# Enigmatisms/NeRF

Measured on AMD Instinct MI355X. Metric: rays/s (64+128 samples), 800x800, higher is better.
Workload: dtype bf16

## Files before the change

### nerf_amd/csrc/host_common.h

```cpp
#pragma once
#include <hip/hip_runtime.h>
#include <mutex>
#include <vector>

namespace nerf_host {

inline std::mutex& table_mutex() { static std::mutex m; return m; }

inline int current_device() {
    int dev = 0;
    if (hipGetDevice(&dev) != hipSuccess) dev = 0;
    return dev;
}

inline int allow_dynamic_lds(const void* fn, size_t lds) {
    struct Entry { int dev; const void* fn; size_t lds; };
    static std::vector<Entry> done;
    const int dev = current_device();
    std::lock_guard<std::mutex> lock(table_mutex());
    for (auto& e : done)
        if (e.dev == dev && e.fn == fn) {
            if (e.lds >= lds) return 0;
            hipError_t err = hipFuncSetAttribute(fn, hipFuncAttributeMaxDynamicSharedMemorySize, (int)lds);
            if (err != hipSuccess) return (int)err;
            e.lds = lds;
            return 0;
        }
    hipError_t err = hipFuncSetAttribute(fn, hipFuncAttributeMaxDynamicSharedMemorySize, (int)lds);
    if (err != hipSuccess) return (int)err;
    done.push_back({dev, fn, lds});
    return 0;
}

inline int cu_count() {
    static int n_cu[64] = {0};
    const int dev = current_device();
    std::lock_guard<std::mutex> lock(table_mutex());
    int& slot = n_cu[dev & 63];
    if (!slot) {
        hipDeviceProp_t p;
        slot = (hipGetDeviceProperties(&p, dev) == hipSuccess && p.multiProcessorCount > 0) ? p.multiProcessorCount : 256;
    }
    return slot;
}

}
```

### nerf_amd/csrc/mlp_kernels.hip

```cpp
#include "mlp_core.h"
#include "launchers.h"

namespace {

template <class P, int L, int NKG>
DEVINL void encode(float x, float y, float z, int h, typename P::BReg (&B)[NKG]) {
    if constexpr (P::FAST_PE) {
        float sv[3], cv[3];
        sincos_quadrant(x, sv[0], cv[0]); sincos_quadrant(y, sv[1], cv[1]); sincos_quadrant(z, sv[2], cv[2]);
#pragma unroll
        for (int f = 0; f < L; ++f) {
#pragma unroll
            for (int c = 0; c < 3; ++c) {
                const int q = 3 * f + c;
                P::set(B[q >> 3], q & 7, h ? cv[c] : sv[c]);
                if (f + 1 < L) {
                    const float s2 = 2.0f * sv[c];
                    const float ns = s2 * cv[c];
                    const float nc = __builtin_fmaf(-s2, sv[c], 1.0f);
                    sv[c] = ns; cv[c] = nc;
                }
            }
        }
#pragma unroll
// ... 233 lines not shown
    split_sample_index(s, m0, q, r);
    n = wave_uniform(q); si0 = __builtin_amdgcn_readfirstlane(r);
}
template <bool EXPLICIT_Z>
DEVINL Sample fetch_ray_sample(const nerf_amd_samples& s, int64_t n, int si) {
    Sample r;
    const float* ry = s.rays + n * 6;
    const float ox = ry[0], oy = ry[1], oz = ry[2];
    r.dx = ry[3]; r.dy = ry[4]; r.dz = ry[5];
    float zv;
    if (EXPLICIT_Z || s.z) zv = s.z[n * s.z_stride + si];
    else {
        const float uu = s.u ? s.u[n * s.S + si] : philox_u_strat(s.rng_seed, n + s.rng_ray_offset, si);
        zv = s.z_base[si] + uu * s.z_jitter;
    }
    r.x = ox + zv * r.dx; r.y = oy + zv * r.dy; r.z = oz + zv * r.dz;
    return r;
}

struct PropResident {
    using R = ResidentSet<PropLayout::N_FRAGS, 32, 0, 168, MLP_RES_PROP_HOLE>;
    static constexpr int NSLOT = MLP_RES_PROP_NSLOT;
    static constexpr uint32_t RING = NSLOT * MLP_CHUNK_BYTES, BIAS = RING, RES = RING + 9216, TOTAL = RES + R::N * 1024;
    static_assert(TOTAL <= 160 * 1024, "LDS");
};
struct MipResident {
    using R = ResidentSet<MipLayout::N_FRAGS, 32, MLP_RES_MIP_TAIL>;
    static constexpr int NSLOT = MLP_RES_MIP_NSLOT;
    static constexpr uint32_t RING = NSLOT * MLP_CHUNK_BYTES, BIAS = RING, STASH = BIAS + MipLayout::N_BIAS * 4, DIR = STASH + 4 * 2 * 4 * 1024,
                              RES = DIR + 4 * 2 * 1024, TOTAL = RES + R::N * 1024;
    static_assert(TOTAL <= 160 * 1024, "LDS");
};

DEVINL void load_biases(const void* packed, size_t stream_bytes, int n_bias, uint32_t lds_off = MLP_RING_BYTES) {
    const float* b = reinterpret_cast<const float*>(reinterpret_cast<const char*>(packed) + stream_bytes);
    float* dst = reinterpret_cast<float*>(smem + lds_off);
    for (int i = threadIdx.x; i < n_bias; i += blockDim.x) dst[i] = b[i];
    __syncthreads();
}

struct ActDump {
    char* base;
    unsigned long long layer_stride;
    char* mask_base;
    unsigned long long mask_layer_stride;
};
template <class P>
DEVINL void dump_breg(const ActDump& d, int layer, int64_t subtile, int kg, int lane, const typename P::BReg& r) {
#ifndef ABL_NODUMPST
    P::store_global(d.base + (size_t)layer * d.layer_stride + ((size_t)subtile * 16 + kg) * (size_t)P::BREG_LDS, lane, r);
#endif
}

template <class P> constexpr uint32_t lds_maskacc() { return lds_total<P>(); }
template <class P> constexpr uint32_t lds_total_train() { return lds_total<P>() + P::NW * 2 * P::NT * 1024; }
template <class P> constexpr uint32_t lds_scaleacc() { return lds_total_train<P>(); }
template <class P> constexpr uint32_t lds_total_train_f8() { return lds_total_train<P>() + P::NW * 2 * P::NT * 1024; }
template <class P, bool F8>
DEVINL void dump_hidden(const ActDump& d, uint32_t sacc_wave, int layer, int64_t subtile, int t, int kg, int lane, const typename P::BReg& r) {
    if constexpr (F8) {
        const uint32_t E = f8_group_exponent<false>(r);
        f8_store_group(d.base + (size_t)layer * d.layer_stride + (size_t)subtile * F8_SUB_BYTES, kg, lane, f8_encode_group(r, E), E,
                       sacc_wave + ((layer & 1) * P::NT + t) * 1024);
    } else {
        dump_breg<P>(d, layer, subtile, kg, lane, r);
    }
// ... 14 lines not shown
DEVINL uint32_t breg_bits(const f32x8& v) {
    uint32_t m = 0;
#pragma unroll
    for (int e = 0; e < 8; ++e) m |= (v[e] > 0.0f ? 1u : 0u) << ((e >> 1) + 16 * (e & 1));
    return m;
}
template <class P>
DEVINL void mask_or(uint32_t acc_wave, int layer, int t, int kg, int lane, const typename P::BReg& v) {
    unsigned* w = reinterpret_cast<unsigned*>(smem + acc_wave + ((layer & 1) * P::NT + t) * 1024 + lane * 16 + (kg >> 2) * 4);
    __hip_atomic_fetch_or(w, breg_bits(v) << (4 * (kg & 3)), __ATOMIC_RELAXED, __HIP_MEMORY_SCOPE_WORKGROUP);
}
template <class P, bool F8 = false>
DEVINL void mask_flush(const ActDump& d, uint32_t acc_wave, int layer, int64_t sub0, int lane, uint32_t sacc_wave = 0) {
    asm volatile("" ::: "memory");
#pragma unroll
    for (int t = 0; t < P::NT; ++t) {
        f32x4* rec = reinterpret_cast<f32x4*>(smem + acc_wave + ((layer & 1) * P::NT + t) * 1024 + lane * 16);
        const f32x4 v = *rec;
        *reinterpret_cast<f32x4*>(d.mask_base + (size_t)layer * d.mask_layer_stride + (size_t)(sub0 + t) * 1024 + lane * 16) = v;
        *rec = f32x4{0.0f, 0.0f, 0.0f, 0.0f};
        if constexpr (F8)
            f8_flush_scales(d.base + (size_t)layer * d.layer_stride + (size_t)(sub0 + t) * F8_SUB_BYTES, lane, sacc_wave + ((layer & 1) * P::NT + t) * 1024);
    }
    asm volatile("" ::: "memory");
}
template <class P>
DEVINL void mask_acc_init(uint32_t acc_wave, int lane) {
#pragma unroll
    for (int i = 0; i < 2 * P::NT; ++i) *reinterpret_cast<f32x4*>(smem + acc_wave + i * 1024 + lane * 16) = f32x4{0.0f, 0.0f, 0.0f, 0.0f};
}

template <class P, bool TRAIN, bool F8 = false>
__global__ __launch_bounds__(P::NW * 64) void proposal_kernel(const void* __restrict__ packed, nerf_amd_samples s,
                                                              float* __restrict__ density, ActDump dump) {
    using L = PropLayout;
    using BReg = typename P::BReg;
    constexpr int FPC = P::FPC;
    constexpr bool RES = MLP_RESIDENT_PROP && wide_bf16<P>() && !TRAIN;
    using R = typename conditional_type<RES, PropResident::R, NoResident>::type;
    using WS = typename conditional_type<RES, WeightStream<P, PropResident::NSLOT, R, PropResident::RES>, WeightStream<P, MLP_NSLOT>>::type;
    constexpr uint32_t bias0 = RES ? PropResident::BIAS : MLP_RING_BYTES;
    load_biases(packed, L::stream_bytes(P::PREC), L::N_BIAS, bias0);
    WS ws;
    ws.init(packed, (L::N_FRAGS - R::N) / FPC);
    const int lane = lane_id(), h = lane >> 5, j = lane & 31;
    const int wave = __builtin_amdgcn_readfirstlane((int)(threadIdx.x >> 6));
    constexpr int NT = P::NT;
    constexpr int TS = P::NW * NT * 32;
    const int64_t n_tiles = (s.M + TS - 1) / TS;
    const uint32_t macc = lds_maskacc<P>() + wave * 2 * NT * 1024;
    const uint32_t sacc = lds_scaleacc<P>() + wave * 2 * NT * 1024;
    if constexpr (TRAIN) mask_acc_init<P>(macc, lane);

    for (int64_t tile = blockIdx.x; tile < n_tiles; tile += gridDim.x) {
        int64_t m[NT];
        BReg enc[NT][4];
        if constexpr (ray_tile<P>::value) {
            static_assert(NT == 2 && P::FAST_PE && !TRAIN, "the ray tile is an inference form of the wide bf16 tile");
            const int64_t m0 = tile * TS + wave * 64;
            int64_t n; int si0;
            split_wave_index(s, m0 < s.M ? m0 : s.M - 64, n, si0);
            const Sample sm = fetch_ray_sample<false>(s, n, si0 + lane);
            encode_pair<P, 10, 4>(sm.x, sm.y, sm.z, enc[0], enc[1]);
            half_swap_groups<4>(enc[0], enc[1]);
        } else if constexpr (NT == 2 && P::FAST_PE) {
            m[0] = tile * TS + (wave * NT) * 32 + j;
            m[1] = m[0] + 32;
            const int64_t mo = h ? m[1] : m[0];
            const Sample sm = fetch_sample(s, mo < s.M ? mo : s.M - 1, false);
            encode_pair<P, 10, 4>(sm.x, sm.y, sm.z, enc[0], enc[1]);
            half_swap_groups<4>(enc[0], enc[1]);
            if constexpr (TRAIN) {
#pragma unroll
                for (int t = 0; t < NT; ++t)
#pragma unroll
                    for (int k = 0; k < 4; ++k) dump_breg<P>(dump, 4, tile * (TS / 32) + wave * NT + t, k, lane, enc[t][k]);
            }
        } else {
#pragma unroll
        for (int t = 0; t < NT; ++t) {
            m[t] = tile * TS + (wave * NT + t) * 32 + j;
            const Sample sm = fetch_sample(s, m[t] < s.M ? m[t] : s.M - 1, false);
            encode<P, 10, 4>(sm.x, sm.y, sm.z, h, enc[t]);
            if constexpr (TRAIN) {
#pragma unroll
                for (int k = 0; k < 4; ++k) dump_breg<P>(dump, 4, tile * (TS / 32) + wave * NT + t, k, lane, enc[t][k]);
            }
        }
        }
        BReg a[NT][16], b[NT][16];
        int lay = 0, lay_pend = 0;
        const int64_t sub0 = tile * (TS / 32) + wave * NT;
        auto put = [&](BReg (&buf)[NT][16], int layer, int fb, int t, const f32x16& acc, int half) {
            buf[t][2 * fb + half] = to_breg_half<P, true>(acc, half);
            if constexpr (TRAIN) {
                dump_hidden<P, F8>(dump, sacc, layer, sub0 + t, t, 2 * fb + half, lane, buf[t][2 * fb + half]);
                mask_or<P>(macc, layer, t, 2 * fb + half, lane, buf[t][2 * fb + half]);
            }
        };
        auto OA = [&](int fb, int t, const f32x16& acc, int half) { put(a, lay, fb, t, acc, half); };
        auto OB = [&](int fb, int t, const f32x16& acc, int half) { put(b, lay, fb, t, acc, half); };
        auto OA_pend = [&](int fb, int t, const f32x16& acc, int half) { put(a, lay_pend, fb, t, acc, half); };
        auto OB_pend = [&](int fb, int t, const f32x16& acc, int half) { put(b, lay_pend, fb, t, acc, half); };
        auto IN_A = [&](int kg, int t) -> BReg { return a[t][kg]; };
        Deferred<P, 6, 2> d = dense<P, 4, 8, L::START[0]>(ws, bias0 + L::BIAS_OFF[0] * 4,
            [&](int kg, int t) -> BReg { return enc[t][kg]; }, OA, NoPrev{});
        static_assert(same_stream_shape<R, FPC>(L::START[1], L::START[3], 128 + P::DEPTH), "chunk parity (in stream space) of the shared a -> b instance");
        auto IN_B = [&](int kg, int t) -> BReg { return b[t][kg]; };
#pragma unroll 1
        for (int r = 0; r < 2; ++r) {
            lay_pend = lay; lay = 1 + 2 * r;
            d = dense<P, 16, 8, L::START[1]>(ws, bias0 + (L::BIAS_OFF[1] + r * 512) * 4, IN_A, OB, prev_of(d, OA_pend));
            if constexpr (TRAIN) mask_flush<P, F8>(dump, macc, lay_pend, sub0, lane, sacc);
            if (r == 0) {
                lay_pend = lay; lay = 2;
                d = dense<P, 16, 8, L::START[2]>(ws, bias0 + L::BIAS_OFF[2] * 4, IN_B, OA, prev_of(d, OB_pend));
                if constexpr (TRAIN) mask_flush<P, F8>(dump, macc, lay_pend, sub0, lane, sacc);
            }
        }
        lay_pend = lay;
        float dens[NT];
        auto OH = [&](int, int t, const f32x16& acc, int half) { if (half == 0) dens[t] = acc[0]; };
        dense<P, 16, 1, L::START[4]>(ws, bias0 + L::BIAS_OFF[4] * 4, IN_B, OH, prev_of(d, OB_pend)).flush(OH);
        if constexpr (TRAIN) mask_flush<P, F8>(dump, macc, lay_pend, sub0, lane, sacc);
#pragma unroll
        for (int t = 0; t < NT; ++t) {
            if constexpr (ray_tile<P>::value) {
                const int64_t m0 = tile * TS + wave * 64;
                if (h == 0 && m0 < s.M) density[m0 + t * 32 + j] = dens[t];
            } else {
                if (h == 0 && m[t] < s.M) density[m[t]] = dens[t];
            }
        }
    }
    ws.drain();
}

constexpr uint32_t lds_total_narrow() { return MLP_RING_BYTES + 9216; }
template <class P>
__global__ __launch_bounds__(P::NW * 64) void proposal128_kernel(const void* __restrict__ packed, nerf_amd_samples s, float* __restrict__ density) {
    using L = PropLayout128;
    using BReg = typename P::BReg;
    constexpr int HK = L::HK, HFB = L::HFB;
    load_biases(packed, L::stream_bytes(P::PREC), L::N_BIAS);
    WeightStream<P, MLP_NSLOT> ws;
    ws.init(packed, L::N_FRAGS / P::FPC);
    const int lane = lane_id(), h = lane >> 5, j = lane & 31;
    const int wave = __builtin_amdgcn_readfirstlane((int)(threadIdx.x >> 6));
    constexpr int NT = P::NT;
    constexpr int TS = P::NW * NT * 32;
    const int64_t n_tiles = (s.M + TS - 1) / TS;
    const uint32_t bias0 = MLP_RING_BYTES;
    for (int64_t tile = blockIdx.x; tile < n_tiles; tile += gridDim.x) {
        int64_t m[NT];
        BReg a[NT][HK], b[NT][HK];
        auto OA = [&](int fb, int t, const f32x16& acc, int half) { a[t][2 * fb + half] = to_breg_half<P, true>(acc, half); };
        auto OB = [&](int fb, int t, const f32x16& acc, int half) { b[t][2 * fb + half] = to_breg_half<P, true>(acc, half); };
        auto IN_A = [&](int kg, int t) -> BReg { return a[t][kg]; };
        auto IN_B = [&](int kg, int t) -> BReg { return b[t][kg]; };
        Deferred<P, HFB - 2, 2> d;
        {
            BReg enc[NT][4];
            constexpr int PAIRED = (NT >= 2 && P::FAST_PE) ? 2 : 0;
#pragma unroll
            for (int t = 0; t < NT; ++t) m[t] = tile * TS + (wave * NT + t) * 32 + j;
            if constexpr (PAIRED) {
                const int64_t mo = h ? m[1] : m[0];
                const Sample sm = fetch_sample(s, mo < s.M ? mo : s.M - 1, false);
// ... 1 lines not shown
                half_swap_groups<4>(enc[0], enc[1]);
            }
#pragma unroll
            for (int t = PAIRED; t < NT; ++t) {
                const Sample sm = fetch_sample(s, m[t] < s.M ? m[t] : s.M - 1, false);
                encode<P, 10, 4>(sm.x, sm.y, sm.z, h, enc[t]);
            }
            d = dense<P, 4, HFB, L::START[0]>(ws, bias0 + L::BIAS_OFF[0] * 4, [&](int kg, int t) -> BReg { return enc[t][kg]; }, OA, NoPrev{});
        }
        d = dense<P, HK, HFB, L::START[1]>(ws, bias0 + L::BIAS_OFF[1] * 4, IN_A, OB, prev_of(d, OA));
        d = dense<P, HK, HFB, L::START[2]>(ws, bias0 + L::BIAS_OFF[2] * 4, IN_B, OA, prev_of(d, OB));
        d = dense<P, HK, HFB, L::START[3]>(ws, bias0 + L::BIAS_OFF[3] * 4, IN_A, OB, prev_of(d, OA));
        float dens[NT];
        auto OH = [&](int, int t, const f32x16& acc, int half) { if (half == 0) dens[t] = acc[0]; };
        dense<P, HK, 1, L::START[4]>(ws, bias0 + L::BIAS_OFF[4] * 4, IN_B, OH, prev_of(d, OB)).flush(OH);
        skip_frags<P, L::USED_FRAGS, L::N_FRAGS - L::USED_FRAGS>(ws);
#pragma unroll
        for (int t = 0; t < NT; ++t)
            if (h == 0 && m[t] < s.M) density[m[t]] = dens[t];
    }
    ws.drain();
}

struct FusedComposite {
    float* rgb;
    float* depth;
    float* weights;
    int white_bkg;
    float near, far;
};

template <class P, bool TRAIN, bool IPE = false, bool F8 = false, bool FUSED = false>
__global__ __launch_bounds__(P::NW * 64) void mip_kernel(const void* __restrict__ packed, nerf_amd_samples s,
                                                         float* __restrict__ rgbo, FusedComposite fc, ActDump dump) {
    using L = MipLayout;
    using BReg = typename P::BReg;
    constexpr int FPC = P::FPC;
#ifdef MLP_CLOCKPROBE
    const uint64_t probe_c0 = __builtin_readcyclecounter(), probe_r0 = __builtin_amdgcn_s_memrealtime();
#endif
    if constexpr (FUSED) { if (threadIdx.x < 16) reinterpret_cast<unsigned*>(smem + lds_tile<P>() + P::NW * P::NT * 32 * 32 + P::NW * P::NT * 8)[threadIdx.x] = 0u; }
    constexpr bool RES = MLP_RESIDENT_MIP && wide_bf16<P>() && !TRAIN && !IPE && !F8 && !FUSED;
    using R = typename conditional_type<RES, MipResident::R, NoResident>::type;
    using WS = typename conditional_type<RES, WeightStream<P, MipResident::NSLOT, R, MipResident::RES>, WeightStream<P, MLP_NSLOT>>::type;
    constexpr uint32_t bias0 = RES ? MipResident::BIAS : LDS_BIAS;
    constexpr uint32_t stash_lds = RES ? MipResident::STASH : LDS_STASH, dirs_lds = RES ? MipResident::DIR : lds_dir<P>();
    load_biases(packed, L::stream_bytes(P::PREC), L::N_BIAS, bias0);
    WS ws;
    ws.init(packed, (L::N_FRAGS - R::N) / FPC);
    const int lane = lane_id(), h = lane >> 5, j = lane & 31;
    const int wave = __builtin_amdgcn_readfirstlane((int)(threadIdx.x >> 6));
    constexpr int NT = P::NT;
    constexpr int TS = P::NW * NT * 32;
    const int64_t n_tiles = (s.M + TS - 1) / TS;
    const uint32_t macc = lds_maskacc<P>() + wave * 2 * NT * 1024;
    const uint32_t sacc = lds_scaleacc<P>() + wave * 2 * NT * 1024;
    if constexpr (TRAIN) mask_acc_init<P>(macc, lane);
    const uint32_t enc_lds0 = stash_lds + wave * NT * 4 * P::BREG_LDS + lane * 16;
    const uint32_t dir_lds0 = dirs_lds + wave * NT * 1024 + lane * 16;
    auto enc_lds = [&](int t) -> uint32_t { return enc_lds0 + t * 4 * P::BREG_LDS; };
    auto dir_lds = [&](int t) -> uint32_t { return dir_lds0 + t * 1024; };

    for (int64_t tile = blockIdx.x; tile < n_tiles; tile += gridDim.x) {
        int64_t m[NT];
        BReg a[NT][16], b[NT][16];
        int lay = 0, lay_pend = 0;
        const int64_t sub0 = tile * (TS / 32) + wave * NT;
        auto put = [&](BReg (&buf)[NT][16], int layer, int fb, int t, const f32x16& acc, int half) {
            buf[t][2 * fb + half] = to_breg_half<P, true>(acc, half);
            if constexpr (TRAIN) {
                dump_hidden<P, F8>(dump, sacc, layer, sub0 + t, t, 2 * fb + half, lane, buf[t][2 * fb + half]);
                mask_or<P>(macc, layer, t, 2 * fb + half, lane, buf[t][2 * fb + half]);
            }
        };
        auto OA = [&](int fb, int t, const f32x16& acc, int half) { put(a, lay, fb, t, acc, half); };
        auto OB = [&](int fb, int t, const f32x16& acc, int half) { put(b, lay, fb, t, acc, half); };
        auto OA_pend = [&](int fb, int t, const f32x16& acc, int half) { put(a, lay_pend, fb, t, acc, half); };
        auto OB_pend = [&](int fb, int t, const f32x16& acc, int half) { put(b, lay_pend, fb, t, acc, half); };
        auto IN_A = [&](int kg, int t) -> BReg { return a[t][kg]; };
        Deferred<P, 6, 2> d;
        {
            BReg enc[NT][4];
            if constexpr (ray_tile<P>::value) {
                static_assert(NT == 2 && P::FAST_PE && !TRAIN && !IPE && !F8 && !FUSED, "the ray tile is an inference form of the wide bf16 tile");
                const int64_t m0 = tile * TS + wave * 64;
                int64_t n; int si0;
                const int64_t m0c = m0 < s.M ? m0 : s.M - 64;
                split_wave_index(s, m0c, n, si0);
                const BReg* row = reinterpret_cast<const BReg*>(reinterpret_cast<const char*>(rgbo + m0c * 4) + h * (DIR_TABLE_ROW / 2));
                const BReg row0 = row[0], row1 = row[1];
                const Sample sm = fetch_ray_sample<true>(s, n, si0 + lane);
                P::stash(dir_lds(0), row0);
                P::stash(dir_lds(1), row1);
                encode_pair<P, 10, 4>(sm.x, sm.y, sm.z, enc[0], enc[1]);
                half_swap_groups<4>(enc[0], enc[1]);
#pragma unroll
                for (int t = 0; t < NT; ++t) {
#pragma unroll
                    for (int k = 0; k < 4; ++k) P::stash(enc_lds(t) + k * P::BREG_LDS, enc[t][k]);
                }
            } else if constexpr (NT == 2 && P::FAST_PE && !IPE && !FUSED) {
                m[0] = tile * TS + (wave * NT) * 32 + j;
                m[1] = m[0] + 32;
                const int64_t mo = h ? m[1] : m[0];
                const Sample sm = fetch_sample(s, mo < s.M ? mo : s.M - 1, true);
                encode_pair<P, 10, 4>(sm.x, sm.y, sm.z, enc[0], enc[1]);
                half_swap_groups<4>(enc[0], enc[1]);
                uint32_t d0[3] = {__builtin_bit_cast(uint32_t, sm.dx), __builtin_bit_cast(uint32_t, sm.dy), __builtin_bit_cast(uint32_t, sm.dz)};
                uint32_t d1[3] = {d0[0], d0[1], d0[2]};
#pragma unroll
                for (int c = 0; c < 3; ++c) half_swap(d0[c], d1[c]);
#pragma unroll
                for (int t = 0; t < NT; ++t) {
#pragma unroll
                    for (int k = 0; k < 4; ++k) P::stash(enc_lds(t) + k * P::BREG_LDS, enc[t][k]);
                    if constexpr (TRAIN) {
#pragma unroll
                        for (int k = 0; k < 4; ++k) dump_breg<P>(dump, 8, sub0 + t, k, lane, enc[t][k]);
                    }
                    const uint32_t* dd = t ? d1 : d0;
                    const f32x4 dv = {__builtin_bit_cast(float, dd[0]), __builtin_bit_cast(float, dd[1]), __builtin_bit_cast(float, dd[2]), 0.0f};
                    *reinterpret_cast<f32x4*>(smem + dir_lds(t)) = dv;
                }
            } else {
#pragma unroll
            for (int t = 0; t < NT; ++t) {
                m[t] = tile * TS + (wave * NT + t) * 32 + j;
                Sample sm;
                if constexpr (IPE) {
                    const IpeSample is = fetch_sample_ipe(s, m[t] < s.M ? m[t] : s.M - 1);
                    encode_ipe<P, 10, 4>(is.mu, is.var, h, enc[t]);
                    sm.dx = is.dx; sm.dy = is.dy; sm.dz = is.dz;
                } else {
                    sm = fetch_sample(s, m[t] < s.M ? m[t] : s.M - 1, true);
                    encode<P, 10, 4>(sm.x, sm.y, sm.z, h, enc[t]);
                }
#pragma unroll
                for (int k = 0; k < 4; ++k) P::stash(enc_lds(t) + k * P::BREG_LDS, enc[t][k]);
                if constexpr (TRAIN) {
#pragma unroll
                    for (int k = 0; k < 4; ++k) dump_breg<P>(dump, 8, sub0 + t, k, lane, enc[t][k]);
                }
                f32x4 dv = {sm.dx, sm.dy, sm.dz, 0.0f};
                if constexpr (FUSED) {
                    const int64_t mm_ = m[t] < s.M ? m[t] : s.M - 1;
                    const int64_t n_ = mm_ / s.S;
                    const int si_ = (int)(mm_ - n_ * s.S);
                    const float nrm_ = norm3(sm.dx, sm.dy, sm.dz);
                    const float* zz_ = s.z + n_ * s.z_stride;
                    const float zn0 = zz_[si_] * nrm_;
                    const float dl = (si_ + 1 < s.S) ? (zz_[si_ + 1] * nrm_ - zn0) : 1e10f;
                    dv[3] = h ? dl : zn0;
                }
                *reinterpret_cast<f32x4*>(smem + dir_lds(t)) = dv;
            }
            }
            d = dense<P, 4, 8, L::START[0]>(ws, bias0 + L::BIAS_OFF[0] * 4,
                [&](int kg, int t) -> BReg { return enc[t][kg]; }, OA, NoPrev{});
        }
        static_assert(same_stream_shape<R, FPC>(L::START[1], L::START[3], 128 + P::DEPTH) && same_stream_shape<R, FPC>(L::START[1], L::START[5], 128 + P::DEPTH) &&
                      same_stream_shape<R, FPC>(L::START[2], L::START[6], 128 + P::DEPTH) && L::BIAS_OFF[6] == 6 * 256, "uniform layer loop (chunk parity in stream space)");
        auto IN_B = [&](int kg, int t) -> BReg { return b[t][kg]; };
#pragma unroll 1
        for (int r = 0; r < 3; ++r) {
            lay_pend = lay; lay = 1 + 2 * r;
            d = dense<P, 16, 8, L::START[1]>(ws, bias0 + (1 + 2 * r) * 256 * 4, IN_A, OB, prev_of(d, OA_pend));
            if constexpr (TRAIN) mask_flush<P, F8>(dump, macc, lay_pend, sub0, lane, sacc);
            lay_pend = lay; lay = 2 + 2 * r;
            if (r == 1) {
                d = dense<P, 20, 8, L::START[4]>(ws, bias0 + L::BIAS_OFF[4] * 4,
                    [&](int kg, int t) -> BReg { if (kg < 4) return P::unstash(enc_lds(t) + kg * P::BREG_LDS); return b[t][kg >= 4 ? kg - 4 : 0]; },
                    OA, prev_of(d, OB_pend));
            } else {
                d = dense<P, 16, 8, L::START[2]>(ws, bias0 + (2 + 2 * r) * 256 * 4, IN_B, OA, prev_of(d, OB_pend));
            }
            if constexpr (TRAIN) mask_flush<P, F8>(dump, macc, lay_pend, sub0, lane, sacc);
        }
        lay_pend = lay;
        float sigma[NT];
        auto OSIG = [&](int, int t, const f32x16& acc, int half) { if (half == 0) sigma[t] = acc[0]; };
        const auto dsig = dense<P, 16, 1, L::START[7]>(ws, bias0 + L::BIAS_OFF[7] * 4, IN_A, OSIG, prev_of(d, OA_pend));
        if constexpr (TRAIN) mask_flush<P, F8>(dump, macc, 6, sub0, lane, sacc);
        BReg denc[NT][2];
        if constexpr (ray_tile<P>::value) {
        } else {
#pragma unroll
        for (int t = 0; t < NT; ++t) {
            const f32x4 dv = *reinterpret_cast<const f32x4*>(smem + dir_lds(t));
            const float nrm = norm3(dv[0], dv[1], dv[2]);
// ... 94 lines not shown
                    const int q = base + lane;
                    const int sg0 = seg0 + (base >> 5);
                    const bool two = base + 32 < S;
                    const double T0 = t_seg[sg0], T1 = two ? t_seg[sg0 + (two ? 1 : 0)] : 1.0;
                    float w = 0.0f;
                    f32x4 ca = {0.0f, 0.0f, 0.0f, 0.0f};
                    float zn = 0.0f;
                    if (q < S) {
                        const int ts = seg0 * 32 + q;
                        ca = t_ca[ts];
                        const u32x4 pz = t_pz[ts];
                        const u32x2 eb = {pz[0], pz[1]};
                        double excl = __builtin_bit_cast(double, eb);
                        if (h) excl = excl * T0;
                        zn = __builtin_bit_cast(float, (uint32_t)pz[2]);
                        w = ca[3] * (float)(carry * excl);
                    }
                    carry *= (T1 * T0);
                    if (q < S) {
                        ar += w * ca[0]; ag += w * ca[1]; abl += w * ca[2]; aw += w; ad += w * zn;
                        if (wout) wout[q] = w;
                    }
                }
                ar = wave_sum(ar); ag = wave_sum(ag); abl = wave_sum(abl); aw = wave_sum(aw); ad = wave_sum(ad);
                if (lane == 0) {
                    if (fc.white_bkg) { const float bg = 1.0f - aw; ar += bg; ag += bg; abl += bg; }
                    fc.rgb[n * 3] = ar; fc.rgb[n * 3 + 1] = ag; fc.rgb[n * 3 + 2] = abl;
                    if (fc.depth) fc.depth[n] = (ad - fc.near) / (fc.far - fc.near);
                }
            }
        }
    }
    ws.drain();
#ifdef MLP_CLOCKPROBE
    if (blockIdx.x == 0 && threadIdx.x == 0 && rgbo != nullptr) {
        reinterpret_cast<uint64_t*>(rgbo)[0] = __builtin_readcyclecounter() - probe_c0;
        reinterpret_cast<uint64_t*>(rgbo)[1] = __builtin_amdgcn_s_memrealtime() - probe_r0;
    }
#endif
}


template <class P>
__global__ __launch_bounds__(P::NW * 64) void mip128_kernel(const void* __restrict__ packed, nerf_amd_samples s, float* __restrict__ rgbo) {
    using L = MipLayout128;
    using BReg = typename P::BReg;
    load_biases(packed, L::stream_bytes(P::PREC), L::N_BIAS);
    WeightStream<P, MLP_NSLOT> ws;
    ws.init(packed, L::N_FRAGS / P::FPC);
    const int lane = lane_id(), h = lane >> 5, j = lane & 31;
    const int wave = __builtin_amdgcn_readfirstlane((int)(threadIdx.x >> 6));
    constexpr int NT = P::NT;
    constexpr int TS = P::NW * NT * 32;
    const int64_t n_tiles = (s.M + TS - 1) / TS;
    const uint32_t bias0 = LDS_BIAS;
    const uint32_t enc_lds0 = LDS_STASH + wave * NT * 4 * P::BREG_LDS + lane * 16;
    const uint32_t dir_lds0 = lds_dir<P>() + wave * NT * 1024 + lane * 16;
    auto enc_lds = [&](int t) -> uint32_t { return enc_lds0 + t * 4 * P::BREG_LDS; };
    auto dir_lds = [&](int t) -> uint32_t { return dir_lds0 + t * 1024; };
    auto bias = [&](int l) -> uint32_t { return bias0 + L::BIAS_OFF[l] * 4; };
    for (int64_t tile = blockIdx.x; tile < n_tiles; tile += gridDim.x) {
        int64_t m[NT];
        BReg a[NT][8], b[NT][8], g[NT][16];
        auto OA = [&](int fb, int t, const f32x16& acc, int half) { a[t][2 * fb + half] = to_breg_half<P, true>(acc, half); };
        auto OB = [&](int fb, int t, const f32x16& acc, int half) { b[t][2 * fb + half] = to_breg_half<P, true>(acc, half); };
        auto OG = [&](int fb, int t, const f32x16& acc, int half) { g[t][2 * fb + half] = to_breg_half<P, true>(acc, half); };
// ... 341 lines not shown
            }
        }
    }
    ws.drain();
}

#if MLP_TU == 0 || MLP_TU == 2
__global__ __launch_bounds__(256) void dir_table_kernel(const float* __restrict__ rays, int64_t n_rows, int rows_per_ray, int row_stride, char* __restrict__ out) {
    using P = PBF16W;
    const int64_t i = (int64_t)blockIdx.x * 256 + threadIdx.x;
    const int64_t r = i >> 1;
    const int h = (int)(i & 1);
    if (r >= n_rows) return;
    const float* ry = rays + (r / rows_per_ray) * 6;
    const float dx = ry[3], dy = ry[4], dz = ry[5];
    const float nrm = norm3(dx, dy, dz);
    P::BReg denc[2];
    encode<P, 4, 2>(dx / nrm, dy / nrm, dz / nrm, h, denc);
    P::BReg* row = reinterpret_cast<P::BReg*>(out + r * row_stride + h * (DIR_TABLE_ROW / 2));
    row[0] = denc[0];
    row[1] = denc[1];
}
#endif

bool ray_tile_descriptor(const nerf_amd_samples& s) { return s.mode == 1 && !s.contract && !s.ipe && s.S > 0 && s.S % 64 == 0 && s.M % s.S == 0; }

int grid_for(int64_t n_tiles) {
    const int n_cu = nerf_host::cu_count();
    return (int)(n_tiles < n_cu ? n_tiles : n_cu);
}

int allow_dynamic_lds(const void* fn, size_t lds) { return nerf_host::allow_dynamic_lds(fn, lds); }

template <class P, class Lay, bool TRAIN = false, bool F8 = false, size_t LDS_FIXED = 0, class K, class... Extra>
int launch(K kernel, const void* packed, const nerf_amd_samples& s, float* out, hipStream_t st, Extra... extra) {
    constexpr int TS = P::NW * P::NT * 32;
    const int64_t n_tiles = (s.M + TS - 1) / TS;
    if (n_tiles == 0) return 0;
    const size_t lds = LDS_FIXED ? LDS_FIXED : (F8 ? lds_total_train_f8<P>() : (TRAIN ? lds_total_train<P>() : lds_total<P>()));
    if (int e = allow_dynamic_lds(reinterpret_cast<const void*>(kernel), lds)) return e;
    hipLaunchKernelGGL(kernel, dim3(grid_for(n_tiles)), dim3(P::NW * 64), lds, st, packed, s, out, extra...);
    return (int)hipGetLastError();
}
const ActDump NO_DUMP{nullptr, 0ull, nullptr, 0ull};

using PB16 = PBF16W;

}

#ifndef MLP_TU
#define MLP_TU 0
#endif
#if MLP_TU == 0 || MLP_TU == 1
int nk::mlp_launch_proposal(const void* packed, int precision, const nerf_amd_samples& s, float* density, hipStream_t st) {
#if MLP_RAY_TILE_PROP
    if (precision == NERF_AMD_BF16 && ray_tile_descriptor(s))
        return launch<PBF16WR, PropLayout, false, false, (MLP_RESIDENT_PROP ? PropResident::TOTAL : 0)>(proposal_kernel<PBF16WR, false>, packed, s, density, st, NO_DUMP);
#endif
    if (precision == NERF_AMD_BF16)
        return launch<PB16, PropLayout, false, false, (MLP_RESIDENT_PROP ? PropResident::TOTAL : 0)>(proposal_kernel<PB16, false>, packed, s, density, st, NO_DUMP);
    return launch<PF32, PropLayout>(proposal_kernel<PF32, false>, packed, s, density, st, NO_DUMP);
}
#endif
#if MLP_TU == 0 || MLP_TU == 2
static int launch_dir_rows(const float* rays, int64_t n_rows, int rows_per_ray, int row_stride, void* out, hipStream_t st) {
    if (n_rows <= 0) return 0;
    hipLaunchKernelGGL(dir_table_kernel, dim3((unsigned)((2 * n_rows + 255) / 256)), dim3(256), 0, st, rays, n_rows, rows_per_ray, row_stride, reinterpret_cast<char*>(out));
    return (int)hipGetLastError();
}
int nk::mlp_launch_dir_table(const float* rays, int64_t N, void* table, hipStream_t st) { return launch_dir_rows(rays, N, 1, DIR_TABLE_ROW, table, st); }
int nk::mlp_launch_mip(const void* packed, int precision, const nerf_amd_samples& s, float* rgbo, hipStream_t st) {
    const FusedComposite off{nullptr, nullptr, nullptr, 0, 0.0f, 1.0f};
#if MLP_RAY_TILE_MIP
    if (precision == NERF_AMD_BF16 && s.z && ray_tile_descriptor(s)) {
        if (int e = launch_dir_rows(s.rays, s.M / 64, s.S / 64, 64 * 16, rgbo, st)) return e;
        return launch<PBF16WR, MipLayout, false, false, (MLP_RESIDENT_MIP ? MipResident::TOTAL : 0)>(mip_kernel<PBF16WR, false>, packed, s, rgbo, st, off, NO_DUMP);
    }
#endif
    if (s.ipe) {
        if (precision == NERF_AMD_BF16) return launch<PB16, MipLayout>(mip_kernel<PB16, false, true>, packed, s, rgbo, st, off, NO_DUMP);
        return launch<PF32, MipLayout>(mip_kernel<PF32, false, true>, packed, s, rgbo, st, off, NO_DUMP);
    }
    if (precision == NERF_AMD_BF16)
        return launch<PB16, MipLayout, false, false, (MLP_RESIDENT_MIP ? MipResident::TOTAL : 0)>(mip_kernel<PB16, false>, packed, s, rgbo, st, off, NO_DUMP);
    return launch<PF32, MipLayout>(mip_kernel<PF32, false>, packed, s, rgbo, st, off, NO_DUMP);
}
int nk::mlp_launch_mip128(const void* packed, int precision, const nerf_amd_samples& s, float* rgbo, hipStream_t st) {
    if (precision == NERF_AMD_BF16) return launch<PB16, MipLayout128>(mip128_kernel<PB16>, packed, s, rgbo, st);
    return launch<PF32, MipLayout128>(mip128_kernel<PF32>, packed, s, rgbo, st);
}
int nk::mlp_launch_mip_composite(const void* packed, int precision, const nerf_amd_samples& s, float* rgb, float* depth, float* weights,
                             int white_bkg, float near, float far, hipStream_t st) {
    const FusedComposite fc{rgb, depth, weights, white_bkg, near, far};
    if (precision == NERF_AMD_BF16) return launch<PB16, MipLayout>(mip_kernel<PB16, false, false, false, true>, packed, s, (float*)nullptr, st, fc, NO_DUMP);
    return launch<PF32, MipLayout>(mip_kernel<PF32, false, false, false, true>, packed, s, (float*)nullptr, st, fc, NO_DUMP);
}
#endif
static ActDump make_dump(void* dump, int precision, int64_t M, int slots) {
    const unsigned long long ls = nk::mlp_train_layer_stride(precision, M);
    return ActDump{reinterpret_cast<char*>(dump), ls, reinterpret_cast<char*>(dump) + (size_t)slots * ls, (unsigned long long)nk::mlp_train_mask_stride(precision, M)};
}
#if MLP_TU == 0 || MLP_TU == 1
template <class P>
static int launch_proposal128(const void* packed, const nerf_amd_samples& s, float* density, hipStream_t st) {
    constexpr int TS = P::NW * P::NT * 32;
    const int64_t n_tiles = (s.M + TS - 1) / TS;
    if (n_tiles == 0) return 0;
    const size_t lds = lds_total_narrow();
    if (int e = allow_dynamic_lds(reinterpret_cast<const void*>(proposal128_kernel<P>), lds)) return e;
    hipLaunchKernelGGL(proposal128_kernel<P>, dim3(grid_for(n_tiles)), dim3(P::NW * 64), lds, st, packed, s, density);
    return (int)hipGetLastError();
}
int nk::mlp_launch_proposal128(const void* packed, int precision, const nerf_amd_samples& s, float* density, hipStream_t st) {
    if (precision == NERF_AMD_BF16) return launch_proposal128<PBF16N>(packed, s, density, st);
    return launch_proposal128<PF32>(packed, s, density, st);
}
int64_t nk::mlp_train_n_sub(int precision, int64_t M) {
    const int64_t ts = (precision != NERF_AMD_F32) ? (int64_t)PB16::NW * PB16::NT * 32 : (int64_t)PF32::NW * PF32::NT * 32;
    return ((M + ts - 1) / ts) * (ts / 32);
}
size_t nk::mlp_train_layer_stride(int precision, int64_t M) { return (size_t)mlp_train_n_sub(precision, M) * 16 * (precision != NERF_AMD_F32 ? 1024 : 2048); }
size_t nk::mlp_train_mask_stride(int precision, int64_t M) { return (size_t)mlp_train_n_sub(precision, M) * 1024; }
int nk::mlp_launch_proposal_train(const void* packed, int precision, const nerf_amd_samples& s, float* density, void* dump, hipStream_t st) {
    if (precision == NERF_AMD_BF16_F8) {
        const ActDump d8 = make_dump(dump, NERF_AMD_BF16, s.M, PROP_DUMP_SLOTS);
        return launch<PB16, PropLayout, true, true>(proposal_kernel<PB16, true, true>, packed, s, density, st, d8);
    }
    const ActDump d = make_dump(dump, precision, s.M, PROP_DUMP_SLOTS);
    if (precision == NERF_AMD_BF16) return launch<PBF16, PropLayout, true>(proposal_kernel<PBF16, true>, packed, s, density, st, d);
    return launch<PF32, PropLayout, true>(proposal_kernel<PF32, true>, packed, s, density, st, d);
}
#endif
#if MLP_TU == 0 || MLP_TU == 2
int nk::mlp_launch_mip_train(const void* packed, int precision, const nerf_amd_samples& s, float* rgbo, void* dump, hipStream_t st) {
    const FusedComposite off{nullptr, nullptr, nullptr, 0, 0.0f, 1.0f};
    if (precision == NERF_AMD_BF16_F8) {
        const ActDump d8 = make_dump(dump, NERF_AMD_BF16, s.M, MIP_DUMP_SLOTS);
        if (s.ipe) return launch<PB16, MipLayout, true, true>(mip_kernel<PB16, true, true, true>, packed, s, rgbo, st, off, d8);
        return launch<PB16, MipLayout, true, true>(mip_kernel<PB16, true, false, true>, packed, s, rgbo, st, off, d8);
    }
    const ActDump d = make_dump(dump, precision, s.M, MIP_DUMP_SLOTS);
    if (s.ipe) {
        if (precision == NERF_AMD_BF16) return launch<PB16, MipLayout, true>(mip_kernel<PB16, true, true>, packed, s, rgbo, st, off, d);
        return launch<PF32, MipLayout, true>(mip_kernel<PF32, true, true>, packed, s, rgbo, st, off, d);
    }
    if (precision == NERF_AMD_BF16) return launch<PB16, MipLayout, true>(mip_kernel<PB16, true>, packed, s, rgbo, st, off, d);
    return launch<PF32, MipLayout, true>(mip_kernel<PF32, true>, packed, s, rgbo, st, off, d);
}

#endif
#if MLP_TU == 0 || MLP_TU == 3
template <class P, bool TRAIN>
static int launch_ref(const void* packed, const nerf_amd_samples& s, float* rgbo, float* normal, const float* bn_noise, ActDump dump, float* aux,
                      int flags, hipStream_t st, unsigned long long seed = 0, const unsigned long long* seed_dev = nullptr, float noise_std = 0.0f) {
    constexpr int TS = P::NW * P::NT * 32;
    const int64_t n_tiles = (s.M + TS - 1) / TS;
    if (n_tiles == 0) return 0;
    const size_t lds = ref_lds_total<P>();
    if (int e = allow_dynamic_lds(reinterpret_cast<const void*>(ref_kernel<P, TRAIN>), lds)) return e;
    hipLaunchKernelGGL((ref_kernel<P, TRAIN>), dim3(grid_for(n_tiles)), dim3(P::NW * 64), lds, st, packed, s, rgbo, normal, bn_noise, dump, aux, flags, seed, seed_dev, noise_std);
    return (int)hipGetLastError();
}
int nk::mlp_launch_ref(const void* packed, int precision, const nerf_amd_samples& s, float* rgbo, float* normal, const float* bn_noise,
                   int flags, hipStream_t st) {
    if (precision == NERF_AMD_BF16) return launch_ref<PB16, false>(packed, s, rgbo, normal, bn_noise, NO_DUMP, nullptr, flags, st);
    return launch_ref<PF32, false>(packed, s, rgbo, normal, bn_noise, NO_DUMP, nullptr, flags, st);
}
int nk::mlp_launch_ref_train(const void* packed, int precision, const nerf_amd_samples& s, float* rgbo, float* normal, const float* bn_noise,
                         void* dump, float* aux, int flags, hipStream_t st, unsigned long long seed, const unsigned long long* seed_dev, float noise_std) {
    const ActDump d = make_dump(dump, precision, s.M, REF_DUMP_SLOTS);
#ifndef REF_TRAIN_WIDE
    if (precision == NERF_AMD_BF16) return launch_ref<PBF16, true>(packed, s, rgbo, normal, bn_noise, d, aux, flags, st, seed, seed_dev, noise_std);
#endif
    if (precision == NERF_AMD_BF16) return launch_ref<PB16, true>(packed, s, rgbo, normal, bn_noise, d, aux, flags, st, seed, seed_dev, noise_std);
    return launch_ref<PF32, true>(packed, s, rgbo, normal, bn_noise, d, aux, flags, st, seed, seed_dev, noise_std);
}
#endif
```

Baseline: 9.670 million.

## Add atomic work-stealing tile queue to bf16 inference proposal and mip kernels

Replaces the static grid-stride tile loop in the wide bf16 inference proposal and mip kernels with a dynamic tile queue. One thread per block atomically increments a global counter to claim its next tile, parks the result in an LDS double-buffered word, and the block reads it on the next iteration. The goal is to balance load across CUs and XCDs when tile times vary. In exchange it adds a per-stream counter pool, a memset before each launch and one global atomic per tile. An optional compile-time tile timing probe is also added.

```diff
diff --git a/nerf_amd/csrc/host_common.h b/nerf_amd/csrc/host_common.h
--- a/nerf_amd/csrc/host_common.h
+++ b/nerf_amd/csrc/host_common.h
@@ -44,4 +44,35 @@
     return slot;
 }
 
+constexpr int TILE_COUNTER_SLOTS = 32;
+constexpr size_t TILE_COUNTER_STRIDE = 128;
+constexpr size_t TILE_COUNTER_POOL_BYTES = TILE_COUNTER_SLOTS * TILE_COUNTER_STRIDE;
+inline int tile_counter(hipStream_t st, unsigned** counter) {
+    struct Pool { int dev; char* base; int used; hipStream_t owner[TILE_COUNTER_SLOTS]; };
+    static std::vector<Pool> pools;
+    const int dev = current_device();
+    std::lock_guard<std::mutex> lock(table_mutex());
+    Pool* p = nullptr;
+    for (auto& q : pools)
+        if (q.dev == dev) p = &q;
+    if (!p) {
+        void* mem = nullptr;
+        if (hipError_t err = hipMalloc(&mem, TILE_COUNTER_POOL_BYTES)) return (int)err;
+        pools.push_back(Pool{dev, reinterpret_cast<char*>(mem), 0, {}});
+        p = &pools.back();
+    }
+    int k = 0;
+    while (k < p->used && p->owner[k] != st) ++k;
+    if (k == p->used) {
+        if (p->used == TILE_COUNTER_SLOTS) {
+            if (hipError_t err = hipDeviceSynchronize()) return (int)err;
+            p->used = 0;
+            k = 0;
+        }
+        p->owner[p->used++] = st;
+    }
+    *counter = reinterpret_cast<unsigned*>(p->base + (size_t)k * TILE_COUNTER_STRIDE);
+    return 0;
 }
+
+}
diff --git a/nerf_amd/csrc/mlp_kernels.hip b/nerf_amd/csrc/mlp_kernels.hip
--- a/nerf_amd/csrc/mlp_kernels.hip
+++ b/nerf_amd/csrc/mlp_kernels.hip
@@ -289,6 +289,79 @@
     static_assert(TOTAL <= 160 * 1024, "LDS");
 };
 
+template <bool ON> struct TileProbe {
+    unsigned tiles;
+    DEVINL void begin() { tiles = 0u; }
+    DEVINL void end() {}
+};
+#ifndef MLP_TILEPROBE
+constexpr bool TILEPROBE = false;
+#else
+constexpr bool TILEPROBE = true;
+constexpr int TILEPROBE_LAUNCHES = 8, TILEPROBE_WGS = 1024;
+struct TileProbeRec {
+    unsigned long long real0, real1;
+    unsigned long long clk0, clk1;
+    unsigned xcc, tiles, grid, seq;
+};
+__device__ TileProbeRec g_tileprobe[TILEPROBE_LAUNCHES][TILEPROBE_WGS];
+__device__ unsigned g_tileprobe_seq;
+__global__ void tileprobe_advance() { g_tileprobe_seq = g_tileprobe_seq + 1; }
+template <> struct TileProbe<true> {
+    unsigned long long real0, clk0;
+    unsigned tiles;
+    DEVINL void begin() { real0 = __builtin_amdgcn_s_memrealtime(); clk0 = __builtin_amdgcn_s_memtime(); tiles = 0u; }
+    DEVINL void end() {
+        const unsigned long long real1 = __builtin_amdgcn_s_memrealtime(), clk1 = __builtin_amdgcn_s_memtime();
+        unsigned xcc;
+        asm volatile("s_getreg_b32 %0, hwreg(HW_REG_XCC_ID)" : "=s"(xcc));
+        if (threadIdx.x == 0 && blockIdx.x < TILEPROBE_WGS) {
+            const unsigned seq = g_tileprobe_seq;
+            g_tileprobe[seq % TILEPROBE_LAUNCHES][blockIdx.x] = TileProbeRec{real0, real1, clk0, clk1, xcc & 0xfu, tiles, gridDim.x, seq};
+        }
+    }
+};
+int tileprobe_read(void* dst, size_t bytes) {
+    if (bytes != sizeof(g_tileprobe)) return (int)hipErrorInvalidValue;
+    if (hipError_t e = hipDeviceSynchronize()) return (int)e;
+    return (int)hipMemcpyFromSymbol(dst, HIP_SYMBOL(g_tileprobe), bytes);
+}
+#endif
+
+#ifndef MLP_ELASTIC
+#define MLP_ELASTIC 1
+#endif
+template <bool ON> struct TileQueue {
+    DEVINL void init(unsigned*, uint32_t) {}
+    DEVINL void fetch() {}
+    DEVINL void park() {}
+    DEVINL int64_t next(int64_t tile) { return tile + gridDim.x; }
+};
+template <> struct TileQueue<true> {
+    unsigned* counter;
+    uint32_t word;
+    uint32_t flip;
+    unsigned got;
+    DEVINL void init(unsigned* c, uint32_t lds) { counter = c; word = lds; flip = lds ^ (lds + 4); }
+    DEVINL void fetch() {
+        if (threadIdx.x == 0) {
+            uint32_t zero = 0u;
+            asm volatile("" : "+v"(zero));
+            got = __hip_atomic_fetch_add(counter + zero, 1u, __ATOMIC_RELAXED, __HIP_MEMORY_SCOPE_AGENT);
+        }
+    }
+    DEVINL void park() { if (threadIdx.x == 0) *reinterpret_cast<volatile uint32_t*>(smem + word) = got; }
+    DEVINL int64_t next(int64_t) {
+        asm volatile("" ::: "memory");
+        const uint32_t nx = (uint32_t)__builtin_amdgcn_readfirstlane((int)*reinterpret_cast<volatile uint32_t*>(smem + word));
+        word ^= flip;
+        return (int64_t)gridDim.x + nx;
+    }
+};
+template <class P, bool TRAIN, bool IPE = false, bool F8 = false, bool FUSED = false>
+constexpr bool elastic_tiles() { return MLP_ELASTIC && (same_type<P, PBF16W>::value || same_type<P, PBF16WR>::value) && !TRAIN && !IPE && !F8 && !FUSED; }
+constexpr uint32_t ELASTIC_LDS = 8;
+
 DEVINL void load_biases(const void* packed, size_t stream_bytes, int n_bias, uint32_t lds_off = MLP_RING_BYTES) {
     const float* b = reinterpret_cast<const float*>(reinterpret_cast<const char*>(packed) + stream_bytes);
     float* dst = reinterpret_cast<float*>(smem + lds_off);
@@ -369,10 +442,12 @@
 
 template <class P, bool TRAIN, bool F8 = false>
 __global__ __launch_bounds__(P::NW * 64) void proposal_kernel(const void* __restrict__ packed, nerf_amd_samples s,
-                                                              float* __restrict__ density, ActDump dump) {
+                                                              float* __restrict__ density, ActDump dump, unsigned* tile_counter) {
     using L = PropLayout;
     using BReg = typename P::BReg;
     constexpr int FPC = P::FPC;
+    TileProbe<TILEPROBE && ray_tile<P>::value && !TRAIN> probe;
+    probe.begin();
     constexpr bool RES = MLP_RESIDENT_PROP && wide_bf16<P>() && !TRAIN;
     using R = typename conditional_type<RES, PropResident::R, NoResident>::type;
     using WS = typename conditional_type<RES, WeightStream<P, PropResident::NSLOT, R, PropResident::RES>, WeightStream<P, MLP_NSLOT>>::type;
@@ -388,8 +463,12 @@
     const uint32_t macc = lds_maskacc<P>() + wave * 2 * NT * 1024;
     const uint32_t sacc = lds_scaleacc<P>() + wave * 2 * NT * 1024;
     if constexpr (TRAIN) mask_acc_init<P>(macc, lane);
-
-    for (int64_t tile = blockIdx.x; tile < n_tiles; tile += gridDim.x) {
+    constexpr bool ELASTIC = elastic_tiles<P, TRAIN>();
+    TileQueue<ELASTIC> tq;
+    tq.init(tile_counter, RES ? PropResident::TOTAL : lds_total<P>());
+
+    for (int64_t tile = blockIdx.x; tile < n_tiles; tile = tq.next(tile)) {
+        ++probe.tiles;
         int64_t m[NT];
         BReg enc[NT][4];
         if constexpr (ray_tile<P>::value) {
@@ -398,6 +477,7 @@
             int64_t n; int si0;
             split_wave_index(s, m0 < s.M ? m0 : s.M - 64, n, si0);
             const Sample sm = fetch_ray_sample<false>(s, n, si0 + lane);
+            tq.fetch();
             encode_pair<P, 10, 4>(sm.x, sm.y, sm.z, enc[0], enc[1]);
             half_swap_groups<4>(enc[0], enc[1]);
         } else if constexpr (NT == 2 && P::FAST_PE) {
@@ -405,6 +485,7 @@
             m[1] = m[0] + 32;
             const int64_t mo = h ? m[1] : m[0];
             const Sample sm = fetch_sample(s, mo < s.M ? mo : s.M - 1, false);
+            tq.fetch();
             encode_pair<P, 10, 4>(sm.x, sm.y, sm.z, enc[0], enc[1]);
             half_swap_groups<4>(enc[0], enc[1]);
             if constexpr (TRAIN) {
@@ -414,6 +495,7 @@
                     for (int k = 0; k < 4; ++k) dump_breg<P>(dump, 4, tile * (TS / 32) + wave * NT + t, k, lane, enc[t][k]);
             }
         } else {
+        static_assert(!ELASTIC, "elastic tiles: the wide bf16 prologues");
 #pragma unroll
         for (int t = 0; t < NT; ++t) {
             m[t] = tile * TS + (wave * NT + t) * 32 + j;
@@ -425,6 +507,7 @@
             }
         }
         }
+        tq.park();
         BReg a[NT][16], b[NT][16];
         int lay = 0, lay_pend = 0;
         const int64_t sub0 = tile * (TS / 32) + wave * NT;
@@ -471,6 +554,7 @@
         }
     }
     ws.drain();
+    probe.end();
 }
 
 constexpr uint32_t lds_total_narrow() { return MLP_RING_BYTES + 9216; }
@@ -538,10 +622,12 @@
 
 template <class P, bool TRAIN, bool IPE = false, bool F8 = false, bool FUSED = false>
 __global__ __launch_bounds__(P::NW * 64) void mip_kernel(const void* __restrict__ packed, nerf_amd_samples s,
-                                                         float* __restrict__ rgbo, FusedComposite fc, ActDump dump) {
+                                                         float* __restrict__ rgbo, FusedComposite fc, ActDump dump, unsigned* tile_counter) {
     using L = MipLayout;
     using BReg = typename P::BReg;
     constexpr int FPC = P::FPC;
+    TileProbe<TILEPROBE && ray_tile<P>::value && !TRAIN> probe;
+    probe.begin();
 #ifdef MLP_CLOCKPROBE
     const uint64_t probe_c0 = __builtin_readcyclecounter(), probe_r0 = __builtin_amdgcn_s_memrealtime();
 #endif
@@ -566,8 +652,12 @@
     const uint32_t dir_lds0 = dirs_lds + wave * NT * 1024 + lane * 16;
     auto enc_lds = [&](int t) -> uint32_t { return enc_lds0 + t * 4 * P::BREG_LDS; };
     auto dir_lds = [&](int t) -> uint32_t { return dir_lds0 + t * 1024; };
-
-    for (int64_t tile = blockIdx.x; tile < n_tiles; tile += gridDim.x) {
+    constexpr bool ELASTIC = elastic_tiles<P, TRAIN, IPE, F8, FUSED>();
+    TileQueue<ELASTIC> tq;
+    tq.init(tile_counter, RES ? MipResident::TOTAL : lds_total<P>());
+
+    for (int64_t tile = blockIdx.x; tile < n_tiles; tile = tq.next(tile)) {
+        ++probe.tiles;
         int64_t m[NT];
         BReg a[NT][16], b[NT][16];
         int lay = 0, lay_pend = 0;
@@ -596,6 +686,7 @@
                 const BReg* row = reinterpret_cast<const BReg*>(reinterpret_cast<const char*>(rgbo + m0c * 4) + h * (DIR_TABLE_ROW / 2));
                 const BReg row0 = row[0], row1 = row[1];
                 const Sample sm = fetch_ray_sample<true>(s, n, si0 + lane);
+                tq.fetch();
                 P::stash(dir_lds(0), row0);
                 P::stash(dir_lds(1), row1);
                 encode_pair<P, 10, 4>(sm.x, sm.y, sm.z, enc[0], enc[1]);
@@ -610,6 +701,7 @@
                 m[1] = m[0] + 32;
                 const int64_t mo = h ? m[1] : m[0];
                 const Sample sm = fetch_sample(s, mo < s.M ? mo : s.M - 1, true);
+                tq.fetch();
                 encode_pair<P, 10, 4>(sm.x, sm.y, sm.z, enc[0], enc[1]);
                 half_swap_groups<4>(enc[0], enc[1]);
                 uint32_t d0[3] = {__builtin_bit_cast(uint32_t, sm.dx), __builtin_bit_cast(uint32_t, sm.dy), __builtin_bit_cast(uint32_t, sm.dz)};
@@ -629,6 +721,7 @@
                     *reinterpret_cast<f32x4*>(smem + dir_lds(t)) = dv;
                 }
             } else {
+            static_assert(!ELASTIC, "elastic tiles: the wide bf16 prologues");
 #pragma unroll
             for (int t = 0; t < NT; ++t) {
                 m[t] = tile * TS + (wave * NT + t) * 32 + j;
@@ -661,6 +754,7 @@
                 *reinterpret_cast<f32x4*>(smem + dir_lds(t)) = dv;
             }
             }
+            tq.park();
             d = dense<P, 4, 8, L::START[0]>(ws, bias0 + L::BIAS_OFF[0] * 4,
                 [&](int kg, int t) -> BReg { return enc[t][kg]; }, OA, NoPrev{});
         }
@@ -821,6 +915,7 @@
         }
     }
     ws.drain();
+    probe.end();
 #ifdef MLP_CLOCKPROBE
     if (blockIdx.x == 0 && threadIdx.x == 0 && rgbo != nullptr) {
         reinterpret_cast<uint64_t*>(rgbo)[0] = __builtin_readcyclecounter() - probe_c0;
@@ -1228,17 +1323,36 @@
 
 int allow_dynamic_lds(const void* fn, size_t lds) { return nerf_host::allow_dynamic_lds(fn, lds); }
 
-template <class P, class Lay, bool TRAIN = false, bool F8 = false, size_t LDS_FIXED = 0, class K, class... Extra>
+template <class P, bool TRAIN, class K, class... Args>
+int enqueue(K kernel, int64_t n_tiles, size_t lds, const void* packed, const nerf_amd_samples& s, float* out, hipStream_t st, Args... args) {
+#ifdef MLP_TILEPROBE
+    if constexpr (ray_tile<P>::value && !TRAIN) hipLaunchKernelGGL(tileprobe_advance, dim3(1), dim3(1), 0, st);
+#endif
+    hipLaunchKernelGGL(kernel, dim3(grid_for(n_tiles)), dim3(P::NW * 64), lds, st, packed, s, out, args...);
+    return (int)hipGetLastError();
+}
+template <class P, class Lay, bool TRAIN = false, bool F8 = false, size_t LDS_FIXED = 0, int TILES = -1, class K, class... Extra>
 int launch(K kernel, const void* packed, const nerf_amd_samples& s, float* out, hipStream_t st, Extra... extra) {
     constexpr int TS = P::NW * P::NT * 32;
     const int64_t n_tiles = (s.M + TS - 1) / TS;
     if (n_tiles == 0) return 0;
-    const size_t lds = LDS_FIXED ? LDS_FIXED : (F8 ? lds_total_train_f8<P>() : (TRAIN ? lds_total_train<P>() : lds_total<P>()));
+    constexpr size_t lds = (LDS_FIXED ? LDS_FIXED : (F8 ? lds_total_train_f8<P>() : (TRAIN ? lds_total_train<P>() : lds_total<P>()))) + (TILES == 1 ? ELASTIC_LDS : 0);
+    static_assert(lds <= 160 * 1024, "LDS");
     if (int e = allow_dynamic_lds(reinterpret_cast<const void*>(kernel), lds)) return e;
-    hipLaunchKernelGGL(kernel, dim3(grid_for(n_tiles)), dim3(P::NW * 64), lds, st, packed, s, out, extra...);
-    return (int)hipGetLastError();
+    if constexpr (TILES == 1) {
+        unsigned* counter = nullptr;
+        if (int e = nerf_host::tile_counter(st, &counter)) return e;
+        if (n_tiles > grid_for(n_tiles))
+            if (hipError_t e = hipMemsetAsync(counter, 0, sizeof(unsigned), st)) return (int)e;
+        return enqueue<P, TRAIN>(kernel, n_tiles, lds, packed, s, out, st, extra..., counter);
+    } else if constexpr (TILES == 0) {
+        return enqueue<P, TRAIN>(kernel, n_tiles, lds, packed, s, out, st, extra..., (unsigned*)nullptr);
+    } else {
+        return enqueue<P, TRAIN>(kernel, n_tiles, lds, packed, s, out, st, extra...);
+    }
 }
 const ActDump NO_DUMP{nullptr, 0ull, nullptr, 0ull};
+[[maybe_unused]] unsigned* const STATIC_TILES = nullptr;
 
 using PB16 = PBF16W;
 
@@ -1246,16 +1360,24 @@
 
 #ifndef MLP_TU
 #define MLP_TU 0
+#endif
+#ifdef MLP_TILEPROBE
+#if MLP_TU == 0 || MLP_TU == 1
+extern "C" __attribute__((visibility("default"))) int nerf_amd_tileprobe_read_prop(void* dst, size_t bytes) { return tileprobe_read(dst, bytes); }
+#endif
+#if MLP_TU == 0 || MLP_TU == 2
+extern "C" __attribute__((visibility("default"))) int nerf_amd_tileprobe_read_mip(void* dst, size_t bytes) { return tileprobe_read(dst, bytes); }
+#endif
 #endif
 #if MLP_TU == 0 || MLP_TU == 1
 int nk::mlp_launch_proposal(const void* packed, int precision, const nerf_amd_samples& s, float* density, hipStream_t st) {
 #if MLP_RAY_TILE_PROP
     if (precision == NERF_AMD_BF16 && ray_tile_descriptor(s))
-        return launch<PBF16WR, PropLayout, false, false, (MLP_RESIDENT_PROP ? PropResident::TOTAL : 0)>(proposal_kernel<PBF16WR, false>, packed, s, density, st, NO_DUMP);
+        return launch<PBF16WR, PropLayout, false, false, (MLP_RESIDENT_PROP ? PropResident::TOTAL : 0), (int)elastic_tiles<PBF16WR, false>()>(proposal_kernel<PBF16WR, false>, packed, s, density, st, NO_DUMP);
 #endif
     if (precision == NERF_AMD_BF16)
-        return launch<PB16, PropLayout, false, false, (MLP_RESIDENT_PROP ? PropResident::TOTAL : 0)>(proposal_kernel<PB16, false>, packed, s, density, st, NO_DUMP);
-    return launch<PF32, PropLayout>(proposal_kernel<PF32, false>, packed, s, density, st, NO_DUMP);
+        return launch<PB16, PropLayout, false, false, (MLP_RESIDENT_PROP ? PropResident::TOTAL : 0), (int)elastic_tiles<PB16, false>()>(proposal_kernel<PB16, false>, packed, s, density, st, NO_DUMP);
+    return launch<PF32, PropLayout>(proposal_kernel<PF32, false>, packed, s, density, st, NO_DUMP, STATIC_TILES);
 }
 #endif
 #if MLP_TU == 0 || MLP_TU == 2
@@ -1270,16 +1392,16 @@
 #if MLP_RAY_TILE_MIP
     if (precision == NERF_AMD_BF16 && s.z && ray_tile_descriptor(s)) {
         if (int e = launch_dir_rows(s.rays, s.M / 64, s.S / 64, 64 * 16, rgbo, st)) return e;
-        return launch<PBF16WR, MipLayout, false, false, (MLP_RESIDENT_MIP ? MipResident::TOTAL : 0)>(mip_kernel<PBF16WR, false>, packed, s, rgbo, st, off, NO_DUMP);
+        return launch<PBF16WR, MipLayout, false, false, (MLP_RESIDENT_MIP ? MipResident::TOTAL : 0), (int)elastic_tiles<PBF16WR, false>()>(mip_kernel<PBF16WR, false>, packed, s, rgbo, st, off, NO_DUMP);
     }
 #endif
     if (s.ipe) {
-        if (precision == NERF_AMD_BF16) return launch<PB16, MipLayout>(mip_kernel<PB16, false, true>, packed, s, rgbo, st, off, NO_DUMP);
-        return launch<PF32, MipLayout>(mip_kernel<PF32, false, true>, packed, s, rgbo, st, off, NO_DUMP);
+        if (precision == NERF_AMD_BF16) return launch<PB16, MipLayout>(mip_kernel<PB16, false, true>, packed, s, rgbo, st, off, NO_DUMP, STATIC_TILES);
+        return launch<PF32, MipLayout>(mip_kernel<PF32, false, true>, packed, s, rgbo, st, off, NO_DUMP, STATIC_TILES);
     }
     if (precision == NERF_AMD_BF16)
-        return launch<PB16, MipLayout, false, false, (MLP_RESIDENT_MIP ? MipResident::TOTAL : 0)>(mip_kernel<PB16, false>, packed, s, rgbo, st, off, NO_DUMP);
-    return launch<PF32, MipLayout>(mip_kernel<PF32, false>, packed, s, rgbo, st, off, NO_DUMP);
+        return launch<PB16, MipLayout, false, false, (MLP_RESIDENT_MIP ? MipResident::TOTAL : 0), (int)elastic_tiles<PB16, false>()>(mip_kernel<PB16, false>, packed, s, rgbo, st, off, NO_DUMP);
+    return launch<PF32, MipLayout>(mip_kernel<PF32, false>, packed, s, rgbo, st, off, NO_DUMP, STATIC_TILES);
 }
 int nk::mlp_launch_mip128(const void* packed, int precision, const nerf_amd_samples& s, float* rgbo, hipStream_t st) {
     if (precision == NERF_AMD_BF16) return launch<PB16, MipLayout128>(mip128_kernel<PB16>, packed, s, rgbo, st);
@@ -1288,8 +1410,8 @@
 int nk::mlp_launch_mip_composite(const void* packed, int precision, const nerf_amd_samples& s, float* rgb, float* depth, float* weights,
                              int white_bkg, float near, float far, hipStream_t st) {
     const FusedComposite fc{rgb, depth, weights, white_bkg, near, far};
-    if (precision == NERF_AMD_BF16) return launch<PB16, MipLayout>(mip_kernel<PB16, false, false, false, true>, packed, s, (float*)nullptr, st, fc, NO_DUMP);
-    return launch<PF32, MipLayout>(mip_kernel<PF32, false, false, false, true>, packed, s, (float*)nullptr, st, fc, NO_DUMP);
+    if (precision == NERF_AMD_BF16) return launch<PB16, MipLayout>(mip_kernel<PB16, false, false, false, true>, packed, s, (float*)nullptr, st, fc, NO_DUMP, STATIC_TILES);
+    return launch<PF32, MipLayout>(mip_kernel<PF32, false, false, false, true>, packed, s, (float*)nullptr, st, fc, NO_DUMP, STATIC_TILES);
 }
 #endif
 static ActDump make_dump(void* dump, int precision, int64_t M, int slots) {
@@ -1320,11 +1442,11 @@
 int nk::mlp_launch_proposal_train(const void* packed, int precision, const nerf_amd_samples& s, float* density, void* dump, hipStream_t st) {
     if (precision == NERF_AMD_BF16_F8) {
         const ActDump d8 = make_dump(dump, NERF_AMD_BF16, s.M, PROP_DUMP_SLOTS);
-        return launch<PB16, PropLayout, true, true>(proposal_kernel<PB16, true, true>, packed, s, density, st, d8);
+        return launch<PB16, PropLayout, true, true>(proposal_kernel<PB16, true, true>, packed, s, density, st, d8, STATIC_TILES);
     }
     const ActDump d = make_dump(dump, precision, s.M, PROP_DUMP_SLOTS);
-    if (precision == NERF_AMD_BF16) return launch<PBF16, PropLayout, true>(proposal_kernel<PBF16, true>, packed, s, density, st, d);
-    return launch<PF32, PropLayout, true>(proposal_kernel<PF32, true>, packed, s, density, st, d);
+    if (precision == NERF_AMD_BF16) return launch<PBF16, PropLayout, true>(proposal_kernel<PBF16, true>, packed, s, density, st, d, STATIC_TILES);
+    return launch<PF32, PropLayout, true>(proposal_kernel<PF32, true>, packed, s, density, st, d, STATIC_TILES);
 }
 #endif
 #if MLP_TU == 0 || MLP_TU == 2
@@ -1332,16 +1454,16 @@
     const FusedComposite off{nullptr, nullptr, nullptr, 0, 0.0f, 1.0f};
     if (precision == NERF_AMD_BF16_F8) {
         const ActDump d8 = make_dump(dump, NERF_AMD_BF16, s.M, MIP_DUMP_SLOTS);
-        if (s.ipe) return launch<PB16, MipLayout, true, true>(mip_kernel<PB16, true, true, true>, packed, s, rgbo, st, off, d8);
-        return launch<PB16, MipLayout, true, true>(mip_kernel<PB16, true, false, true>, packed, s, rgbo, st, off, d8);
+        if (s.ipe) return launch<PB16, MipLayout, true, true>(mip_kernel<PB16, true, true, true>, packed, s, rgbo, st, off, d8, STATIC_TILES);
+        return launch<PB16, MipLayout, true, true>(mip_kernel<PB16, true, false, true>, packed, s, rgbo, st, off, d8, STATIC_TILES);
     }
     const ActDump d = make_dump(dump, precision, s.M, MIP_DUMP_SLOTS);
     if (s.ipe) {
-        if (precision == NERF_AMD_BF16) return launch<PB16, MipLayout, true>(mip_kernel<PB16, true, true>, packed, s, rgbo, st, off, d);
-        return launch<PF32, MipLayout, true>(mip_kernel<PF32, true, true>, packed, s, rgbo, st, off, d);
-    }
-    if (precision == NERF_AMD_BF16) return launch<PB16, MipLayout, true>(mip_kernel<PB16, true>, packed, s, rgbo, st, off, d);
-    return launch<PF32, MipLayout, true>(mip_kernel<PF32, true>, packed, s, rgbo, st, off, d);
+        if (precision == NERF_AMD_BF16) return launch<PB16, MipLayout, true>(mip_kernel<PB16, true, true>, packed, s, rgbo, st, off, d, STATIC_TILES);
+        return launch<PF32, MipLayout, true>(mip_kernel<PF32, true, true>, packed, s, rgbo, st, off, d, STATIC_TILES);
+    }
+    if (precision == NERF_AMD_BF16) return launch<PB16, MipLayout, true>(mip_kernel<PB16, true>, packed, s, rgbo, st, off, d, STATIC_TILES);
+    return launch<PF32, MipLayout, true>(mip_kernel<PF32, true>, packed, s, rgbo, st, off, d, STATIC_TILES);
 }
 
 #endif
```

New measurement: 9.767 million (median of 6 runs). +1.0%, better.
